# bcosm/CantorRL

Hardware: AMD Instinct MI355X
Metric: env-steps/sec (batched episodes) (higher is better)
Workload: dtype f64+f32; 1 GPU; configs[1]: 65,536 parallel envs/GPU, European call (BS rolling-ATM marks), GBM, v2 env, train_ppo_v2 reward; config_index=2, envs_per_gpu=65536, episode_length=252, mode=rollout, rollout_k=256, action_sets=1, parallelism=env-shard x1

## Files before the change

### cantorrl_amd/csrc/hedge_env.hip

```cpp
#include <hip/hip_runtime.h>
#include <hip/hip_ext.h>

#include <math.h>
#include <stdarg.h>
#include <stdio.h>
#include <stdlib.h>
#include <string.h>

#include <chrono>
#include <new>
#include <type_traits>

#include "vn_moments.h"
#include <string>
#include <vector>

#include "../../include/hedge_env.h"
#include "he_math.h"

using namespace he;

namespace {

#define GLOBAL __attribute__((address_space(1)))
// ... 1623 lines not shown
                                                          int slot0, vn::MomentsArgs vm) {
    Io io;
    io.act = sio.act;
    io.obs = sio.obs;
    io.rew = sio.rew;
    io.term = sio.term;
    io.trunc = sio.trunc;
    io.tobs = sio.tobs;
    io.info = he_info{};
    io.pol_on = false;
    io.sums = false;
    io.sig = nullptr;
    static_assert(kEpw == 64 && kEpb == kBlock, "one env per thread");
    const int64_t r = (int64_t)blockIdx.x * kEpb + threadIdx.x;
    const double ret_prev = (vm.upd_ret && r < n) ? vm.returns[r] : 0.0;
    const double col_shift = vn::load_col_shift(vm);
    VnHook hk{nullptr, 0.0f, 0.0, false};
    step_body<MODE, false, true, BOOK, FAST, false, GS>(*pc, n, tA, tB, tC, s, io, 1, slot0, blockIdx.x, &hk);
    __syncthreads();
    vn::moments_from_rows(vm, blockIdx.x, hk.tile, hk.rew, ret_prev, col_shift);
}

template <int MODE, bool BOOK, bool FAST, bool GS>
__global__ __launch_bounds__(kBlock) void step1_vne_kernel(const Params* __restrict__ pc, int64_t n, const float4* tA,
                                                           const float4* tB, const double* tC, State s, StepIo sio,
                                                           int slot0, vn::ApplyArgs va) {
    Io io;
    io.act = sio.act;
    io.obs = sio.obs;
    io.rew = sio.rew;
    io.term = sio.term;
    io.trunc = sio.trunc;
    io.tobs = sio.tobs;
    io.info = he_info{};
    io.pol_on = false;
    io.sums = false;
    io.sig = nullptr;
    static_assert(kEpw == 64 && kEpb == kBlock, "one env per thread");
    const int64_t r0 = (int64_t)blockIdx.x * kEpb;
    __shared__ vn::FrozenNorm fz;
    const vn::FrozenPre fp = vn::load_frozen(va, r0 + threadIdx.x, r0 + threadIdx.x < n);
    vn::prep_frozen(fz, va, fp);
    VnHook hk{nullptr, 0.0f, 0.0, false};
    step_body<MODE, false, true, BOOK, FAST, false, GS>(*pc, n, tA, tB, tC, s, io, 1, slot0, blockIdx.x, &hk);
    const int rows = (int)((n - r0) < kEpb ? n - r0 : kEpb);
    __syncthreads();
    vn::apply_frozen_rows(va, fz, r0, rows, hk.tile, fp, hk.rew, hk.rew64, hk.term, sio.tobs);
}

__global__ __launch_bounds__(vn::kVnThreads) void vn_moments_after_step_kernel(vn::MomentsArgs vm) {
    vn::moments_body(vm, blockIdx.x);
}

constexpr int kFusedWaves = kMktWaves;
template <int MODE, bool BOOK, bool FAST, bool GS>
__global__ __launch_bounds__(kBlock, kFusedWaves) void step_market_kernel(const Params* __restrict__ pc, int32_t buf,
                                                                           State s, Io io, int k_steps, int slot0,
                                                                           Market cur, Market bak,
                                                                           int32_t step_blocks) {
    static_assert(kBlock == kMktEnvs * kMktLanes, "one workgroup shape for both roles");
    if ((int32_t)blockIdx.x < step_blocks) {
        const Params& pk = pc[buf];
        step_body<MODE, false, false, BOOK, FAST, false, GS>(pk, pk.n, pk.tileA, pk.tileB, pk.tileC, s, io, k_steps,
                                                              slot0, blockIdx.x);
    } else {
        market_body<MODE, BOOK>(pc[buf ^ 1], cur, bak, 0, (int64_t)blockIdx.x - step_blocks);
    }
}

#ifndef HE_LDS_BALANCE
#define HE_LDS_BALANCE 1
#endif


constexpr int kPrioRewBook = 0, kPrioReplayRew = 0, kPrioObs = 2, kPrioProd = 1;
constexpr int kPrioGbmRew = 3, kPrioGbmObs = 2, kPrioGbmProd0 = 1, kPrioGbmProd1 = 0;
constexpr int kLdsLanesGbm = 2, kLdsLanesBook = 2, kLdsMinWavesBook = 4;
constexpr int kLdsEnvs = 64;
constexpr int kLdsM = 8;
constexpr int kLdsPrefetch = kLdsM % 6 == 0 ? 6 : (kLdsM % 4 == 0 ? 4 : kLdsM);
static_assert(kLdsM % kLdsPrefetch == 0, "the action ring index is the slot mod D");

template <int MODE, bool BOOK>
struct LdsGeom {
    static constexpr bool HESTON = MODE == HE_MODE_HESTON;
    static constexpr int lanes = (BOOK || HESTON) ? kLdsLanesBook : kLdsLanesGbm;
    static constexpr int prod = lanes;
    static constexpr int penvs = kLdsEnvs / lanes;
    static constexpr int threads = 64 * (2 + prod);
    static constexpr int H = kLdsM / lanes;
    static constexpr int minwaves = (BOOK || HESTON) ? kLdsMinWavesBook
                                                     : (HE_LDS_BALANCE ? 4 : (4 * (2 + prod) + 3) / 4 + 1);
    static_assert(H * lanes == kLdsM && penvs * lanes == kLdsEnvs, "producer lane layout");
};

constexpr int kLdsBookRows = 256;
constexpr int lds_thp_rows() { return 512; }
template <int MODE, bool BOOK, bool LEAN = false>
struct LdsMarketT {
    static constexpr int NB = 2;
    static constexpr bool THP = LEAN && !BOOK;
    double thp[THP ? lds_thp_rows() : 1];
    float2 sc[NB][kLdsM][kLdsEnvs];
    float pp[NB][kLdsM][kLdsEnvs];
    float stage[2][kLdsEnvs * kObs];
    double bk[BOOK ? 2 : 1][BOOK ? kLdsM : 1][kLdsEnvs];
    float vv[MODE == HE_MODE_HESTON ? 2 : 1][MODE == HE_MODE_HESTON ? kLdsM : 1][kLdsEnvs];
    double btab[BOOK ? kLdsBookRows : 1][4];
    BookOpt bopt[BOOK ? HE_BOOK_MAX : 1];
    uint32_t tame[NB][2];
};
static_assert(kLdsM > 8 || sizeof(LdsMarketT<HE_MODE_GBM, false>) <= 40 * 1024, "4 workgroups per CU");
static_assert(kLdsM > 8 || sizeof(LdsMarketT<HE_MODE_GBM, false, true>) <= 40 * 1024 - 64, "4 workgroups per CU");
static_assert(kLdsM > 8 || sizeof(LdsMarketT<HE_MODE_HESTON, true>) <= 40 * 1024, "4 workgroups per CU");

#ifdef HE_LDS_TIMING
__device__ uint64_t g_lds_tim[4][4096][5];
#define LDS_T0() uint64_t tim_t0 = __builtin_amdgcn_s_memtime(), tim_bar = 0, tim_r0 = __builtin_amdgcn_s_memrealtime()
#define LDS_BAR()                                                  \
    do {                                                           \
        const uint64_t tb_ = __builtin_amdgcn_s_memtime();         \
        __syncthreads();                                           \
        tim_bar += __builtin_amdgcn_s_memtime() - tb_;             \
    } while (0)
#define LDS_T1(role)                                                                     \
    do {                                                                                 \
        if ((threadIdx.x & 63) == 0 && blockIdx.x < 4096) {                              \
            g_lds_tim[role][blockIdx.x][0] = __builtin_amdgcn_s_memtime() - tim_t0;      \
            g_lds_tim[role][blockIdx.x][1] = tim_bar;                                    \
            const uint64_t r1_ = __builtin_amdgcn_s_memrealtime();                       \
            g_lds_tim[role][blockIdx.x][2] = r1_ - tim_r0;                               \
            g_lds_tim[role][blockIdx.x][3] = tim_r0;                                     \
            g_lds_tim[role][blockIdx.x][4] = r1_;                                        \
        }                                                                                \
    } while (0)
#else
#define LDS_T0() do {} while (0)
#define LDS_BAR() __syncthreads()
#define LDS_T1(role) do {} while (0)
#endif

__device__ __forceinline__ void flush_obs_full(const float* img, float* out, int64_t row0, int lane) {
    asm volatile("" ::: "memory");
    GLOBAL float* dst = (GLOBAL float*)out + row0 * kObs;
    GLOBAL v4f* d4 = (GLOBAL v4f*)dst;
    const v4f* s4 = reinterpret_cast<const v4f*>(img);
    d4[lane] = s4[lane];
    d4[lane + 64] = s4[lane + 64];
    d4[lane + 128] = s4[lane + 128];
    dst[768 + lane] = img[768 + lane];
    asm volatile("" ::: "memory");
}

template <int MODE, bool BOOK, bool LEAN, bool OBS, bool POL = false, bool PLAIN_OK = false, bool TAME_OK = false>
__device__ __forceinline__ void lds_stepper(const Params& p, State s, const Io& io, int k_steps, const Market& cur,
                                            LdsMarketT<MODE, BOOK, LEAN>& L, int64_t base) {
    constexpr int D = kLdsPrefetch;
    constexpr bool HESTON = MODE == HE_MODE_HESTON;
    const int lane = threadIdx.x & 63;
    const int64_t N = p.n;
    const int nfull = k_steps / kLdsM;
    const int tail = k_steps - nfull * kLdsM;
    const int64_t i0 = base + lane;
    const int64_t i = i0 < N ? i0 : N - 1;
    const int wrows = (int)((N - base) < kLdsEnvs ? (N - base) : kLdsEnvs);
    const Mkt rst{p.rstv[0], p.rstv[1], p.rstv[2], p.rstv[3], BOOK ? p.book_rst : 0.0};
    const GLOBAL v2f* gact = (const GLOBAL v2f*)io.act;
    GLOBAL float* const grew = (GLOBAL float*)io.rew;
    GLOBAL uint8_t* const gterm = (GLOBAL uint8_t*)io.term;
    if (!BOOK && !HESTON) {
        if (OBS) __builtin_amdgcn_s_setprio(kPrioGbmObs);
        else __builtin_amdgcn_s_setprio(kPrioGbmRew);
    } else {
        if (OBS) __builtin_amdgcn_s_setprio(kPrioObs);
        else __builtin_amdgcn_s_setprio(kPrioRewBook);
    }
    LDS_T0();
    Env e{};
    Mkt pre = rst;
    double pv_last = 0.0;
    {
        const uint32_t t0 = s.t[i];
        const uint32_t pk = s.pos[i];
        e.t = t0;
        e.call = unpack_lo(pk);
        e.put = unpack_hi(pk);
        e.path = -1;
        e.s0_small = rst.S < 1e-6f;
        e.s0 = e.s0_small ? 1.0f : rst.S;
        if (!OBS) {
            e.cash = s.cash[i];
            if (t0 != 0) {
                const double Sc = cur.S[i];
                const double Vc = HESTON ? cur.v[i] : p.var;
                const double Bc = BOOK ? book_value(p, Sc, Vc, (int32_t)t0, cur.M[i]) : 0.0;
                pre = Mkt{(float)Sc, HESTON ? (float)Vc : p.var_f, cur.C[i], cur.P[i], Bc};
            }
            pv_last = portfolio_value<BOOK>(p, e, pre);
        }
    }
    double sm0 = 0.0, sm1 = 0.0, sm2 = 0.0;
    uint32_t slen = 0;
    float last0 = 0.f, last1 = 0.f, last2 = 0.f, last3 = 0.f;
    if (!OBS) {
        sm0 = s.sum[i];
        sm1 = s.sum[N + i];
        sm2 = s.sum[2 * N + i];
        slen = s.sum_len[i];
        last0 = s.last[i];
        last1 = s.last[N + i];
        last2 = s.last[2 * N + i];
        last3 = s.last[3 * N + i];
    }
    auto account = [&](double reward, double pnl, double tc, bool term) {
        const double a0 = sm0 + reward, a1 = sm1 + pnl, a2 = sm2 + tc;
        const uint32_t n = slen + 1u;
        float f0 = (float)a0, f1 = (float)a1, f2 = (float)a2, f3 = (float)n;
        asm volatile("" : "+v"(f0), "+v"(f1), "+v"(f2), "+v"(f3));
        last0 = term ? f0 : last0;
        last1 = term ? f1 : last1;
        last2 = term ? f2 : last2;
        last3 = term ? f3 : last3;
        sm0 = term ? 0.0 : a0;
        sm1 = term ? 0.0 : a1;
        sm2 = term ? 0.0 : a2;
        slen = term ? 0u : n;
    };
    float2 ra[D];
    if constexpr (!POL) {
#pragma unroll
        for (int d = 0; d < D; ++d) ra[d] = ld2(gact, (int64_t)(d < k_steps ? d : k_steps - 1) * N + i);
    } else {
#pragma unroll
        for (int d = 0; d < D; ++d) ra[d] = make_float2(0.0f, 0.0f);
    }
    const int pol = POL ? io.pol.policy : HE_POLICY_NO_HEDGE;
    const bool pol_greeks = POL && pol != HE_POLICY_NO_HEDGE;
    float po3 = 0.0f, po4 = 0.0f, pcd = 0.0f, ppd = 0.0f;
    double acc[7] = {0.0, 0.0, 0.0, 0.0, 0.0, 0.0, 0.0};
    uint32_t acc_len = 0;
    const bool pmh = LEAN || p.maxh != 0, prm = LEAN || p.record_metrics;
    if constexpr (POL) {
        po3 = pmh ? div_int_byf((float)e.call, p.maxh_f, p.inv_maxh_f) : 0.0f;
        po4 = pmh ? div_int_byf((float)e.put, p.maxh_f, p.inv_maxh_f) : 0.0f;
        if (e.t == 0) {
            pcd = p.rstv[4 + 7];
            ppd = p.rstv[4 + 9];
        } else if (pol_greeks && prm) {
            const float S0f = (float)cur.S[i];
            float4 g0;
            if constexpr (!LEAN) g0 = greeks_fast<!HESTON>(p, S0f, HESTON ? (float)cur.v[i] : p.var_f);
            else if constexpr (HESTON) g0 = greeks_fast<false>(p, S0f, (float)cur.v[i]);
            else g0 = greeks_lean(S0f, p.g_num_drift, p.g_inv_sst_f, p.g_sst_f);
            pcd = g0.x;
            ppd = g0.z;
        }
        if (!OBS) {
#pragma unroll
            for (int c = 0; c < 7; ++c) acc[c] = s.acc[(int64_t)c * N + i];
            acc_len = s.acc_len[i];
        }
    }
    auto pol_account = [&](double reward, double pnl, double ps, double tc, double rpc, double tcp, bool term) {
        acc[0] = acc[0] + reward;
        acc[1] = acc[1] + pnl;
        acc[2] = acc[2] + fabs(ps);
        acc[3] = acc[3] + tc;
        acc[4] = acc[4] + rpc;
        acc[5] = acc[5] + tcp;
        acc[6] = acc[6] + ps;
        acc_len += 1u;
        if (__ballot(term) != 0ull) {
            if (term) {
                if (i0 < N) {
                    const unsigned long long r = atomicAdd(io.pol.count, 1ull);
                    if ((int64_t)r < io.pol.cap) {
                        he_episode_record rec;
                        rec.env_id = p.goff + i;
                        rec.length = (int32_t)acc_len;
                        rec.reserved = 0;
                        rec.reward_sum = acc[0];
                        rec.pnl_sum = acc[1];
                        rec.abs_pnl_sum = acc[2];
                        rec.cost_sum = acc[3];
                        rec.pnl_penalty_sum = acc[4];
                        rec.cost_penalty_sum = acc[5];
                        rec.per_share_pnl_sum = acc[6];
                        rec.reserved2 = 0.0;
                        io.pol.rec[r] = rec;
                    }
                }
                last0 = (float)acc[0];
                last1 = (float)acc[1];
                last2 = (float)acc[3];
                last3 = (float)acc_len;
#pragma unroll
                for (int c = 0; c < 7; ++c) acc[c] = 0.0;
                acc_len = 0;
            }
        }
    };

    constexpr int NB = LdsMarketT<MODE, BOOK, LEAN>::NB;
    constexpr bool kPlain = PLAIN_OK && LEAN && !POL;
    constexpr bool kTame = kPlain && TAME_OK && OBS && MODE == HE_MODE_GBM && !BOOK;
    const bool tame_h = kTame && p.lds_tame != 0;
    auto run_blk = [&](auto&& step, auto&& pre_ok) {
        LDS_BAR();
        for (int b = 0; b < nfull; ++b) {
            const int buf = b % NB;
            auto slots = [&](auto plain) {
#pragma unroll
                for (int sl = 0; sl < kLdsM; ++sl) {
                    const int k = b * kLdsM + sl;
                    const float2 ak = ra[sl % D];
                    if constexpr (!POL) {
                        const int kn = k + D;
                        ra[sl % D] = ld2(gact, (int64_t)(kn < k_steps ? kn : k_steps - 1) * N + i);
                    }
                    step(buf, sl, k, ak, std::true_type{}, plain);
                }
            };
            if constexpr (kPlain) {
                if (__ballot((int32_t)(e.t + (uint32_t)kLdsM) >= p.T) == 0ull) {
                    if constexpr (kTame) {
                        const uint32_t tw = __builtin_amdgcn_readfirstlane(L.tame[buf][0] & L.tame[buf][1]);
                        if (tame_h && tw != 0u && __ballot(!pre_ok()) == 0ull) slots(std::integral_constant<int, 2>{});
                        else slots(std::true_type{});
                    } else {
                        slots(std::true_type{});
                    }
                } else {
                    slots(std::false_type{});
                }
            } else {
                slots(std::false_type{});
            }
            LDS_BAR();
        }
        if (tail) {
            const int buf = nfull % NB;
            for (int sl = 0; sl < tail; ++sl) {
                const int k = nfull * kLdsM + sl;
                step(buf, sl, k, POL ? make_float2(0.0f, 0.0f) : ld2(gact, (int64_t)k * N + i), std::false_type{},
                     std::false_type{});
            }
            LDS_BAR();
        }
    };

    if constexpr (LEAN) {
        const float mt_f = p.mt_f, maxh_f = p.maxh_f, inv_maxh_f = p.inv_maxh_f;
        const int32_t mt = p.mt, maxh = p.maxh, T = p.T;
        if (OBS) {
            const float s0s_f = p.s0s_f, inv_s0s_f = p.inv_s0s_f;
            const float T_f = p.T_f, inv_T_f = p.inv_T_f, var_f = p.var_f;
            const float gnd = p.g_num_drift, gis = p.g_inv_sst_f, gsf = p.g_sst_f;
            float ro[kObs];
#pragma unroll
            for (int c = 0; c < kObs; ++c) ro[c] = p.rstv[4 + c];
            float preS = pre.S;
            if (e.t != 0) preS = (float)cur.S[i];
            const float dv12 = np_clipf(var_f - var_f, -1.0f, 1.0f);
            auto pre_ok = [&] { return preS >= 64.0f && preS <= 8388608.0f; };
            float preV = rst.v;
            if (HESTON && e.t != 0) preV = (float)cur.v[i];
            const double s0s_d = p.s0s_d, inv_s0s_d = p.inv_s0s_d;
            using lds_float = __attribute__((address_space(3))) float;
            lds_float* row0 = (lds_float*)&L.stage[0][lane * kObs];
            lds_float* row1 = (lds_float*)&L.stage[1][lane * kObs];
            asm volatile("" : "+v"(row0), "+v"(row1));
            auto obs_step = [&](int buf, int sl, int k, float2 ak, auto full, auto plain) {
                constexpr bool PLAIN = decltype(plain)::value;
                constexpr bool TAME = (int)decltype(plain)::value == 2;
                const float2 r0 = L.sc[buf][sl][lane];
                const float rP = L.pp[buf][sl][lane];
                const float vk = HESTON ? L.vv[HESTON ? buf : 0][HESTON ? sl : 0][lane] : var_f;
                float4 g;
                if constexpr (HESTON) g = greeks_fast<false>(p, r0.x, vk);
                else g = greeks_lean_t<TAME>(r0.x, gnd, gis, gsf);
                if constexpr (POL) {
                    ak = policy_action(p, pol, e.call, e.put, po3, po4, pcd, ppd);
                    if (io.pol.act_out) {
                        v2f av = {ak.x, ak.y};
                        ((GLOBAL v2f*)io.pol.act_out)[(int64_t)k * N + i] = av;
                    }
                }
                const int32_t nc = e.call + trade_round(ak.x * mt_f, mt);
                const int32_t nq = e.put + trade_round(ak.y * mt_f, mt);
                const int32_t cc = clamp_pos(nc, maxh);
                const int32_t qq = clamp_pos(nq, maxh);
                const uint32_t t1 = e.t + 1;
                const bool term = !PLAIN && (int32_t)t1 >= T;
                float o[kObs];
                if constexpr (TAME) {
                    o[0] = div_f32_byf_nz(r0.x, s0s_f, inv_s0s_f);
                    o[1] = div_f32_by_nz(r0.y, s0s_d, inv_s0s_d);
                    o[2] = div_f32_by_nz(rP, s0s_d, inv_s0s_d);
                } else {
                    if constexpr (HESTON) {
                        o[0] = div_f32_by(r0.x, s0s_d, inv_s0s_d);
                    } else {
                        o[0] = div_f32_byf(r0.x, s0s_f, inv_s0s_f);
                    }
                    o[1] = div_f32_by(r0.y, s0s_d, inv_s0s_d);
                    o[2] = div_f32_by(rP, s0s_d, inv_s0s_d);
                }
                o[3] = div_int_byf((float)cc, maxh_f, inv_maxh_f);
                o[4] = div_int_byf((float)qq, maxh_f, inv_maxh_f);
                o[5] = vk;
                o[6] = div_int_byf((float)(T - (int32_t)t1), T_f, inv_T_f);
                o[7] = g.x;
                o[8] = g.y;
                o[9] = g.z;
                o[10] = g.y;
                o[11] = lag_return_lean<TAME>(r0.x, preS);
                if constexpr (HESTON) o[12] = (preS == 0.0f) ? 0.0f : np_clipf(vk - preV, -1.0f, 1.0f);
                else if constexpr (TAME) o[12] = 0.0f;
                else o[12] = (preS == 0.0f) ? 0.0f : dv12;
                float* const tile = L.stage[k & 1];
                lds_float* const row = (k & 1) ? row1 : row0;
#pragma unroll
                for (int c = 0; c < kObs; ++c) row[c] = o[c];
                if constexpr (!PLAIN) {
                    if (__ballot(term) != 0ull) {
                        if (term) {
#pragma unroll
                            for (int c = 0; c < kObs; ++c) row[c] = ro[c];
                        }
                    }
                }
                if (!POL || io.obs) {
                    float* out = io.obs + (int64_t)k * N * kObs;
                    if constexpr (decltype(full)::value) flush_obs_full(tile, out, base, lane);
                    else flush_obs_wave(tile, out, base, wrows, lane);
                }
                if constexpr (POL) {
                    po3 = term ? ro[3] : o[3];
                    po4 = term ? ro[4] : o[4];
                    pcd = term ? ro[7] : o[7];
                    ppd = term ? ro[9] : o[9];
                }
                e.t = term ? 0u : t1;
                e.call = term ? 0 : cc;
                e.put = term ? 0 : qq;
                preS = term ? rst.S : r0.x;
                if (HESTON) preV = term ? rst.v : vk;
            };
            if (wrows == kLdsEnvs)
                run_blk([&](int buf, int sl, int k, float2 ak, auto, auto plain) {
                    obs_step(buf, sl, k, ak, std::true_type{}, plain);
                }, pre_ok);
            else
                run_blk([&](int buf, int sl, int k, float2 ak, auto, auto plain) {
                    obs_step(buf, sl, k, ak, std::false_type{}, plain);
                }, pre_ok);
        } else {
            const double tcpc = p.tcpc, slip_frac = p.slip_frac, lam = p.lam, w = p.w, theta = p.theta;
            const double shares_d = p.shares_d, inv_shares = p.inv_shares, den = p.den, inv_den = p.inv_den;
            const double inv_252 = p.inv_252, init_cash = p.initial_cash;
// ... 370 lines not shown
                        if (BOOK) Mr = np_max(Mr, S);
                        if (!PLAIN) tp = (tp + 1 == T) ? 0u : tp + 1;
                    }
#pragma unroll
                    for (int h = 0; h < kLdsH; ++h) Sx[h] = (j == sl0 + h) ? S : Sx[h];
                    if (BOOK) {
#pragma unroll
                        for (int h = 0; h < kLdsH; ++h) Mx[h] = (j == sl0 + h) ? Mr : Mx[h];
                    }
                }
            }
            Sbs = S;
            if (BOOK) Mbs = Mr;
            uint32_t tp = tpf;
            const int wb = bp % LdsMarketT<MODE, BOOK, LEAN>::NB;
            double lkC[kLdsH], lkP[kLdsH];
            if constexpr (LOCK) {
                double Sm[kLdsH], Km[kLdsH];
                uint32_t tq = tpf;
#pragma unroll
                for (int h = 0; h < kLdsH; ++h) {
                    if constexpr (PLAIN) {
                        Sm[h] = Sx[h];
                    } else {
                        const bool last = tq + 1 == T;
                        const double Sprev = (h == 0) ? Sin : Sx[h - 1];
                        Sm[h] = last ? ((tq == 0) ? p.s0 : Sprev) : Sx[h];
                        tq = (tq + 1 == T) ? 0u : tq + 1;
                    }
                    Km[h] = rint(Sm[h]);
                }
                bs_call_put_n<kLdsH>(Sm, Km, p.bs, lkC, lkP);
            }
            if constexpr (kTame) {
                uint32_t verdict = 0u;
                if constexpr (LOCK && PLAIN) {
                    uint32_t smin = (uint32_t)__double2hiint(Sx[0]), smax = smin;
                    uint32_t mmin = (uint32_t)__double2hiint(lkC[0]), mmax = mmin;
#pragma unroll
                    for (int h = 0; h < kLdsH; ++h) {
                        const uint32_t sh = (uint32_t)__double2hiint(Sx[h]);
                        const uint32_t ch = (uint32_t)__double2hiint(lkC[h]), ph = (uint32_t)__double2hiint(lkP[h]);
                        smin = sh < smin ? sh : smin;
                        smax = sh > smax ? sh : smax;
                        mmin = ch < mmin ? ch : mmin;
                        mmax = ch > mmax ? ch : mmax;
                        mmin = ph < mmin ? ph : mmin;
                        mmax = ph > mmax ? ph : mmax;
                    }
                    const bool ok = smin >= 0x40500000u && smax < 0x41600000u && mmin >= 0x38100000u && mmax < 0x47e00000u;
                    verdict = __ballot(!ok) == 0ull ? 0xffffffffu : 0u;
                }
                W.tame[wb][pw] = verdict;
            }
            if constexpr (LOCK) {
#pragma unroll
                for (int h = 0; h < kLdsH; ++h) {
                    const int sl = sl0 + h;
                    W.sc[wb][sl][le] = make_float2((float)Sx[h], (float)lkC[h]);
                    W.pp[wb][sl][le] = (float)lkP[h];
                }
            } else {
                double rS[kLdsH], rV[kLdsH];
#pragma unroll
                for (int h = 0; h < kLdsH; ++h) {
                    rS[h] = Sx[h];
                    rV[h] = HESTON ? Vx[h] : p.var;
                }
                double Sprev = Sin, Vprev = Vin;
#pragma unroll 1
                for (int h = 0; h < kLdsH; ++h) {
                    if (FULL || sl0 + h < len) {
                        const bool last = tp + 1 == T;
                        const double Sm = last ? ((tp == 0) ? p.s0 : Sprev) : rS[0];
                        const double Vh = rV[0];
                        const double Vm = HESTON ? (last ? ((tp == 0) ? p.var : Vprev) : Vh) : p.var;
                        float C, P;
                        marks<MODE, !LEAN>(p, Sm, Vm, last ? tp : tp + 1u, &C, &P);
                        const int sl = sl0 + h;
                        W.sc[wb][sl][le] = make_float2((float)rS[0], C);
                        W.pp[wb][sl][le] = P;
                        if (HESTON) W.vv[HESTON ? wb : 0][HESTON ? sl : 0][le] = (float)Vh;
                        tp = (tp + 1 == T) ? 0u : tp + 1;
                    }
                    Sprev = rS[0];
                    Vprev = rV[0];
#pragma unroll
                    for (int q = 0; q + 1 < kLdsH; ++q) {
                        rS[q] = rS[q + 1];
                        rV[q] = rV[q + 1];
                    }
                }
            }
            if constexpr (BOOK) {
                double bS[kLdsH], bV[kLdsH], bM[kLdsH];
#pragma unroll
                for (int h = 0; h < kLdsH; ++h) {
                    bS[h] = Sx[h];
                    bV[h] = HESTON ? Vx[h] : p.var;
                    bM[h] = Mx[h];
                }
                uint32_t tb = tpf;
#pragma unroll 1
                for (int h = 0; h < kLdsH; ++h) {
                    if (HESTON) prod_prio_toggle((h + pw) & 1);
                    else prod_prio_toggle(pw == 1 ? (h != 3) : (h == 3));
                    if (FULL || sl0 + h < len)
                        W.bk[wb][sl0 + h][le] = book_value<!HESTON>(p, bS[0], bV[0], (int32_t)(tb + 1), bM[0],
                                                                    &W.btab[0][0], &W.bopt[0]);
                    tb = (tb + 1 == T) ? 0u : tb + 1;
#pragma unroll
                    for (int q = 0; q + 1 < kLdsH; ++q) {
                        bS[q] = bS[q + 1];
                        bV[q] = bV[q + 1];
                        bM[q] = bM[q + 1];
                    }
                }
            }
            };
            if (len == kLdsM) {
                if constexpr (PLAIN_OK && LEAN && !HESTON && !BOOK) {
                    if (__ballot(tpb == 0u || tpb + (uint32_t)kLdsM >= T) == 0ull)
                        block(std::true_type{}, std::true_type{});
                    else
                        block(std::true_type{}, std::false_type{});
                } else {
                    block(std::true_type{}, std::false_type{});
                }
            } else {
                block(std::false_type{}, std::false_type{});
            }
            tpb = episode_wrap(tpb, (uint32_t)kLdsM, T);
        }
        LDS_BAR();
    }
    if (nb > 0 && sub == 0) {
        const int sll = (k_steps - 1) - (nb - 1) * kLdsM;
        const int wbl = (nb - 1) % LdsMarketT<MODE, BOOK, LEAN>::NB;
        int64_t j = pi;
        asm volatile("" : "+v"(j));
        const uint32_t ep0 = cur.ep[j], t0 = cur.t[j];
        const uint32_t q = (t0 >= T ? T : t0) + (uint32_t)(k_steps - 1);
        cur.ep[j] = ep0 + q / T;
        cur.t[j] = q % T + 1u;
        cur.S[j] = Sbs;
        if (HESTON) cur.v[j] = Vbs;
        cur.C[j] = W.sc[wbl][sll][le].y;
        cur.P[j] = W.pp[wbl][sll][le];
        if (BOOK) cur.M[j] = Mbs;
    }
    LDS_T1(2 + (pw < 2 ? pw : 1));
}

#if HE_LDS_BALANCE || defined(HE_LDS_HWID)
__device__ uint32_t g_cu_ticket[4096];
#endif
#ifdef HE_LDS_HWID
__device__ uint32_t g_lds_hwid[16384][4][4];
#endif
__device__ __forceinline__ uint32_t hw_cu_key(uint32_t hw, uint32_t xcc) {
    return ((xcc & 15u) << 8) | (((hw >> 13) & 7u) << 5) | (((hw >> 12) & 1u) << 4) | ((hw >> 8) & 15u);
}
template <int NWAVES>
__device__ __forceinline__ int lds_role(int wave) {
#if HE_LDS_BALANCE || defined(HE_LDS_HWID)
    if constexpr (NWAVES == 4) {
        __shared__ uint32_t sh_place[5];
        const uint32_t hw = __builtin_amdgcn_s_getreg((31 << 11) | 4);
        const uint32_t xcc = __builtin_amdgcn_s_getreg((15 << 11) | 20);
        const uint32_t simd = (hw >> 4) & 3u;
        if ((threadIdx.x & 63) == 0) sh_place[wave] = simd;
        if (threadIdx.x == 0) sh_place[4] = atomicAdd(&g_cu_ticket[hw_cu_key(hw, xcc & 15u)], 1u);
        __syncthreads();
        const uint32_t m = (1u << sh_place[0]) | (1u << sh_place[1]) | (1u << sh_place[2]) | (1u << sh_place[3]);
        int role = wave;
#if HE_LDS_BALANCE
        if (m == 15u) role = (int)((simd + sh_place[4]) & 3u);
#endif
#ifdef HE_LDS_HWID
        if ((threadIdx.x & 63) == 0 && blockIdx.x < 16384) {
            g_lds_hwid[blockIdx.x][wave][0] = hw;
            g_lds_hwid[blockIdx.x][wave][1] = xcc;
            g_lds_hwid[blockIdx.x][wave][2] = sh_place[4];
            g_lds_hwid[blockIdx.x][wave][3] = (uint32_t)role | (m << 8);
        }
#endif
        return __builtin_amdgcn_readfirstlane(role);
    }
#endif
    return wave;
}

constexpr int kLdsNumSgpr = 96;
constexpr bool kPlainPersistS = false, kPlainPersistP = true;
template <int MODE, bool BOOK, bool LEAN, bool PERSIST = false, bool POL = false>
__global__ __launch_bounds__((LdsGeom<MODE, BOOK>::threads), (LdsGeom<MODE, BOOK>::minwaves))
    __attribute__((amdgpu_num_sgpr(kLdsNumSgpr))) void lds_rollout_kernel(const Params* __restrict__ pc, State s, Io io,
                                                                 int k_steps, Market cur) {
    __shared__ __attribute__((aligned(16))) LdsMarketT<MODE, BOOK, LEAN> lm;
    const Params& p = *pc;
    const int wave = lds_role<LdsGeom<MODE, BOOK>::threads / 64>(__builtin_amdgcn_readfirstlane(threadIdx.x >> 6));
    if constexpr (BOOK) {
        const int nv = 4 * p.book_rows;
        for (int k = threadIdx.x; k < nv; k += LdsGeom<MODE, BOOK>::threads) (&lm.btab[0][0])[k] = p.book_tab[k];
        if ((int)threadIdx.x < p.book_n) lm.bopt[threadIdx.x] = p.book[threadIdx.x];
        __syncthreads();
    }
    if constexpr (!PERSIST) {
        const int64_t base = (int64_t)blockIdx.x * kLdsEnvs;
        if (wave == 0) lds_stepper<MODE, BOOK, LEAN, false, POL, true>(p, s, io, k_steps, cur, lm, base);
        else if (wave == 1) lds_stepper<MODE, BOOK, LEAN, true, POL, true, !POL>(p, s, io, k_steps, cur, lm, base);
        else lds_producer<MODE, BOOK, LEAN, true, !POL>(p, k_steps, cur, lm, base, wave - 2);
        return;
    }
    const int64_t tiles = (p.n + kLdsEnvs - 1) / kLdsEnvs;
    for (int64_t tile = blockIdx.x; tile < tiles; tile += gridDim.x) {
        asm volatile("" ::: "memory");
        const int64_t base = tile * kLdsEnvs;
        if (wave == 0) lds_stepper<MODE, BOOK, LEAN, false, POL, kPlainPersistS>(p, s, io, k_steps, cur, lm, base);
        else if (wave == 1) lds_stepper<MODE, BOOK, LEAN, true, POL, kPlainPersistS>(p, s, io, k_steps, cur, lm, base);
        else lds_producer<MODE, BOOK, LEAN, kPlainPersistP>(p, k_steps, cur, lm, base, wave - 2);
        if (tile + gridDim.x < tiles) __syncthreads();
    }
}

struct LdsReplay {
    float4 mk[2][kLdsM][kLdsEnvs];
    float2 gd[2][kLdsM][kLdsEnvs];
    float gg[2][kLdsM][kLdsEnvs];
    float4 rk[2][kLdsEnvs];
    float4 rg[2][kLdsEnvs];
    float stage[2][kLdsEnvs * kObs];
};
static_assert(kLdsM > 8 || sizeof(LdsReplay) <= 40 * 1024 - 64, "4 workgroups per CU");

__device__ __forceinline__ void lds_replay_loader(const Params& p, State s, int k_steps, LdsReplay& L,
                                                  int64_t base, int part) {
    constexpr int H = kLdsM / 2;
    static_assert(kLdsM == 8, "two lanes per env, 4 slots each: one 128-B line of rows per block");
    const int lane = threadIdx.x & 63;
    const int hh = lane >> 5;
    const int le = part * 32 + (lane & 31);
    const int64_t N = p.n;
    const int64_t i0 = base + le;
    const int64_t i = i0 < N ? i0 : N - 1;
    const uint32_t T = (uint32_t)p.T;
    const int64_t W = p.rstride;
    const GLOBAL v4f* rec = (const GLOBAL v4f*)p.rec;
    const GLOBAL v4f* recg = (const GLOBAL v4f*)p.recg;
    const int sl0 = hh * H;
    __builtin_amdgcn_s_setprio(kPrioProd);
    LDS_T0();
    int32_t path = s.path[i];
    uint32_t t = s.t[i];
    Pcg64 g;
    g.sh = s.pcg[i];
    g.sl = s.pcg[N + i];
    g.ih = s.pcg[2 * N + i];
    g.il = s.pcg[3 * N + i];
    g.has32 = s.pcgb[i];
    g.buf32 = s.pcgb[N + i];
    float s0enc = s.s0[i];
    const int nb = (k_steps + kLdsM - 1) / kLdsM;
    float4 A[H], B[H];
    float4 Y[H];
    bool hand = false;
    float4 R0 = make_float4(0.f, 0.f, 0.f, 0.f), G0 = R0;
    int rsl = kLdsM;
    auto issue = [&](int bp) {
        const int kb = bp * kLdsM;
        const int len = (k_steps - kb) < kLdsM ? (k_steps - kb) : kLdsM;
        const bool take = hand;
        if (__ballot(take) != 0ull) {
#pragma unroll
            for (int h = 0; h < H; ++h) {
                Y[h].x = __shfl(Y[h].x, lane | 32);
                Y[h].y = __shfl(Y[h].y, lane | 32);
                Y[h].z = __shfl(Y[h].z, lane | 32);
                Y[h].w = __shfl(Y[h].w, lane | 32);
            }
        }
        const uint32_t te = T - 1u - t;
        rsl = te < (uint32_t)len ? (int)te : kLdsM;
        int32_t np = path;
        if (rsl < kLdsM) np = (int32_t)pcg64_integers(g, (uint64_t)p.n_paths);
        const int64_t ro = (int64_t)path * W + p.roff + (int64_t)t + 1, rn = (int64_t)np * W + p.roff;
        hand = rsl == kLdsM && (ro & 7) == 4 && t + 12u <= T;
        if (hh == 0 && take) {
#pragma unroll
            for (int h = 0; h < H; ++h) A[h] = Y[h];
        } else {
#pragma unroll
            for (int h = 0; h < H; ++h) {
                const int sl = sl0 + h;
                const int64_t r = (sl <= rsl) ? ro + sl : rn + (sl - rsl);
                A[h] = ld4(rec, r);
            }
        }
        if (hh == 1 && hand) {
#pragma unroll
            for (int h = 0; h < H; ++h) Y[h] = ld4(rec, ro + kLdsM + h);
        }
        if (hh == 0 && rsl < kLdsM) {
            R0 = ld4(rec, rn);
            G0 = ld4(recg, rn);
        }
        if (rsl < kLdsM) {
            path = np;
            t = (uint32_t)(len - 1 - rsl);
        } else {
            t += (uint32_t)len;
        }
    };
    if (nb > 0) issue(0);
    for (int bp = 0; bp <= nb; ++bp) {
        if (bp < nb) {
            const int kb = bp * kLdsM;
            const int len = (k_steps - kb) < kLdsM ? (k_steps - kb) : kLdsM;
            const int wb = bp & 1;
#pragma unroll
            for (int h = 0; h < H; ++h) {
                const int sl = sl0 + h;
                if (sl < len) {
                    B[h] = p.record_metrics ? replay_greeks(p, A[h].x, A[h].y) : make_float4(0.f, 0.f, 0.f, 0.f);
                    L.mk[wb][sl][le] = A[h];
                    L.gd[wb][sl][le] = make_float2(B[h].x, B[h].z);
                    L.gg[wb][sl][le] = B[h].y;
                }
            }
            if (hh == 0) {
                L.rk[wb][le] = R0;
                L.rg[wb][le] = G0;
                if (rsl < kLdsM) s0enc = (R0.x < 1e-6f) ? -1.0f : R0.x;
            }
            if (bp + 1 < nb) issue(bp + 1);
        }
        LDS_BAR();
    }
    LDS_T1(2 + part);
    if (hh == 0 && i0 < N) {
        int64_t j = i;
        asm volatile("" : "+v"(j));
        s.path[j] = path;
        s.s0[j] = s0enc;
        s.pcg[j] = g.sh;
        s.pcg[N + j] = g.sl;
        s.pcgb[j] = g.has32;
        s.pcgb[N + j] = g.buf32;
    }
}

__device__ __forceinline__ uint32_t fresh_lane() {
    uint32_t ln;
    asm volatile("v_mbcnt_lo_u32_b32 %0, -1, 0\n\tv_mbcnt_hi_u32_b32 %0, -1, %0" : "=v"(ln));
    return ln;
}

template <bool OBS, bool FAST, bool POL = false>
__device__ __forceinline__ void lds_replay_stepper(const Params& p, State s, const Io& io, int k_steps,
                                                   LdsReplay& L, int64_t base) {
    constexpr int D = kLdsPrefetch;
    static_assert(kLdsM % D == 0, "the action ring index is the slot mod D");
    const int lane = threadIdx.x & 63;
    const int64_t N = p.n;
    const int nfull = k_steps / kLdsM;
// ... 1938 lines not shown
```

Baseline: 65.73 billion env-steps/s.

## Split GBM LDS producer into pipelined factor-generation and marks-pricing waves

For the plain GBM non-book lean rollout, the two producer waves are replaced by a two-stage pipeline. One wave generates Philox normals and exp growth factors into a double-buffered LDS stage. The other wave consumes those factors to advance the price and compute Black-Scholes marks into the market LDS buffers. The stepper waves take an extra barrier to stay aligned with the deeper pipeline. This aims to overlap RNG/exp work with pricing, at the cost of extra LDS, an extra barrier stage, and a possible occupancy loss.

```diff
diff --git a/cantorrl_amd/csrc/hedge_env.hip b/cantorrl_amd/csrc/hedge_env.hip
--- a/cantorrl_amd/csrc/hedge_env.hip
+++ b/cantorrl_amd/csrc/hedge_env.hip
@@ -1799,7 +1799,8 @@
     asm volatile("" ::: "memory");
 }
 
-template <int MODE, bool BOOK, bool LEAN, bool OBS, bool POL = false, bool PLAIN_OK = false, bool TAME_OK = false>
+template <int MODE, bool BOOK, bool LEAN, bool OBS, bool POL = false, bool PLAIN_OK = false, bool TAME_OK = false,
+          bool STAGE = false>
 __device__ __forceinline__ void lds_stepper(const Params& p, State s, const Io& io, int k_steps, const Market& cur,
                                             LdsMarketT<MODE, BOOK, LEAN>& L, int64_t base) {
     constexpr int D = kLdsPrefetch;
@@ -1953,6 +1954,7 @@
     constexpr bool kTame = kPlain && TAME_OK && OBS && MODE == HE_MODE_GBM && !BOOK;
     const bool tame_h = kTame && p.lds_tame != 0;
     auto run_blk = [&](auto&& step, auto&& pre_ok) {
+        if constexpr (STAGE) LDS_BAR();
         LDS_BAR();
         for (int b = 0; b < nfull; ++b) {
             const int buf = b % NB;
@@ -2629,6 +2631,210 @@
     LDS_T1(2 + (pw < 2 ? pw : 1));
 }
 
+struct LdsStageGf {
+    double gf[2][kLdsM][kLdsEnvs];
+};
+static_assert(kLdsM > 8 || sizeof(LdsMarketT<HE_MODE_GBM, false, true>) + sizeof(LdsStageGf) <= 40 * 1024 - 64,
+              "4 workgroups per CU");
+#ifdef HE_LDS_STAGE_PRIO_SWAP
+constexpr int kPrioStageFactors = kPrioGbmProd0, kPrioStageMarks = kPrioGbmProd1;
+#else
+constexpr int kPrioStageFactors = kPrioGbmProd1, kPrioStageMarks = kPrioGbmProd0;
+#endif
+
+__device__ __forceinline__ void lds_stage_factors(const Params& p, int k_steps, const Market& cur, LdsStageGf& G,
+                                                  int64_t base) {
+    static_assert(kLdsM == 8, "4 Philox blocks (5 from an odd step index) per block of 8 slots");
+    const int lane = threadIdx.x & 63;
+    const int64_t N = p.n;
+    const int nb = (k_steps + kLdsM - 1) / kLdsM;
+    const int64_t pi = (base + lane) < N ? base + lane : N - 1;
+    __builtin_amdgcn_s_setprio(kPrioStageFactors);
+    uint64_t a0;
+    {
+        const uint32_t T = (uint32_t)p.T;
+        const uint32_t ep0 = cur.ep[pi], t0 = cur.t[pi];
+        a0 = (uint64_t)ep0 * T + (t0 >= T ? T : t0);
+    }
+    LDS_T0();
+    for (int bf = 0; bf <= nb + 1; ++bf) {
+        if (bf < nb) {
+            const int64_t gid = p.goff + pi;
+            const uint64_t nf = a0 + (uint64_t)(bf * kLdsM);
+            const uint64_t m0 = nf >> 1;
+            const bool odd = (nf & 1) != 0;
+            double zs[kLdsM];
+            if (__ballot(odd) == 0ull) {
+                philox_normals_n<kLdsM / 2>(p, gid, m0, zs);
+            } else {
+                double zz[kLdsM + 2];
+                philox_normals_n<kLdsM / 2 + 1>(p, gid, m0, zz);
+#pragma unroll
+                for (int j = 0; j < kLdsM; ++j) {
+                    double a = zz[j], b = zz[j + 1];
+                    asm volatile("" : "+v"(a), "+v"(b));
+                    zs[j] = odd ? b : a;
+                }
+            }
+            double arg[kLdsM], ex[kLdsM];
+#pragma unroll
+            for (int j = 0; j < kLdsM; ++j) {
+                const double dW = p.sqrt_dt * zs[j];
+                arg[j] = p.drift + p.sqrt_var * dW;
+            }
+            exp_k_n<4>(arg, ex);
+            exp_k_n<4>(arg + 4, ex + 4);
+            const int wb = bf & 1;
+#pragma unroll
+            for (int j = 0; j < kLdsM; ++j) G.gf[wb][j][lane] = ex[j];
+        }
+        LDS_BAR();
+    }
+    LDS_T1(2);
+}
+
+__device__ __forceinline__ void lds_stage_marks(const Params& p, int k_steps, const Market& cur,
+                                                LdsMarketT<HE_MODE_GBM, false, true>& W, const LdsStageGf& G,
+                                                int64_t base) {
+    constexpr int NB = LdsMarketT<HE_MODE_GBM, false, true>::NB;
+    constexpr int kHalf = kLdsM / 2;
+    const int lane = threadIdx.x & 63;
+    const int64_t N = p.n;
+    const int nb = (k_steps + kLdsM - 1) / kLdsM;
+    const uint32_t T = (uint32_t)p.T;
+    const int64_t pi = (base + lane) < N ? base + lane : N - 1;
+    __builtin_amdgcn_s_setprio(kPrioStageMarks);
+    uint32_t tpb;
+    {
+        const uint32_t t0 = cur.t[pi];
+        tpb = t0 >= T ? 0u : t0;
+    }
+    double Sbs = cur.S[pi];
+    LDS_T0();
+    LDS_BAR();
+    for (int bp = 0; bp <= nb; ++bp) {
+        if (bp < nb) {
+            const int kb = bp * kLdsM;
+            const int len = (k_steps - kb) < kLdsM ? (k_steps - kb) : kLdsM;
+            const int wb = bp % NB;
+            auto block = [&](auto full, auto plain) {
+                constexpr bool FULL = decltype(full)::value;
+                constexpr bool PLAIN = decltype(plain)::value;
+                double eall[kLdsM];
+#pragma unroll
+                for (int j = 0; j < kLdsM; ++j) eall[j] = G.gf[bp & 1][j][lane];
+                const double Sin = Sbs;
+                double Sa[kLdsM];
+                double S = Sbs;
+                uint32_t tp = tpb;
+#pragma unroll
+                for (int j = 0; j < kLdsM; ++j) {
+                    if (FULL || j < len) {
+                        if (!PLAIN && tp == 0) S = p.s0;
+                        const double Sn = S * eall[j];
+                        S = (Sn < 1e-8) ? 1e-8 : Sn;
+                        if (!PLAIN) tp = (tp + 1 == T) ? 0u : tp + 1;
+                    }
+                    Sa[j] = S;
+                }
+                Sbs = S;
+                if constexpr (FULL) {
+                    uint32_t smin = 0xffffffffu, smax = 0u, mmin = 0xffffffffu, mmax = 0u;
+                    uint32_t tq = tpb;
+#pragma unroll
+                    for (int h0 = 0; h0 < kLdsM; h0 += kHalf) {
+                        double Sm[kHalf], Km[kHalf], lkC[kHalf], lkP[kHalf];
+#pragma unroll
+                        for (int h = 0; h < kHalf; ++h) {
+                            const int j = h0 + h;
+                            if constexpr (PLAIN) {
+                                Sm[h] = Sa[j];
+                            } else {
+                                const bool last = tq + 1 == T;
+                                const double Sprev = (j == 0) ? Sin : Sa[j == 0 ? 0 : j - 1];
+                                Sm[h] = last ? ((tq == 0) ? p.s0 : Sprev) : Sa[j];
+                                tq = (tq + 1 == T) ? 0u : tq + 1;
+                            }
+                            Km[h] = rint(Sm[h]);
+                        }
+                        bs_call_put_n<kHalf>(Sm, Km, p.bs, lkC, lkP);
+#pragma unroll
+                        for (int h = 0; h < kHalf; ++h) {
+                            const int j = h0 + h;
+                            if constexpr (PLAIN) {
+                                const uint32_t sh = (uint32_t)__double2hiint(Sa[j]);
+                                const uint32_t ch = (uint32_t)__double2hiint(lkC[h]), ph = (uint32_t)__double2hiint(lkP[h]);
+                                smin = sh < smin ? sh : smin;
+                                smax = sh > smax ? sh : smax;
+                                mmin = ch < mmin ? ch : mmin;
+                                mmax = ch > mmax ? ch : mmax;
+                                mmin = ph < mmin ? ph : mmin;
+                                mmax = ph > mmax ? ph : mmax;
+                            }
+                            W.sc[wb][j][lane] = make_float2((float)Sa[j], (float)lkC[h]);
+                            W.pp[wb][j][lane] = (float)lkP[h];
+                        }
+                    }
+                    uint32_t verdict = 0u;
+                    if constexpr (PLAIN) {
+                        const bool ok = smin >= 0x40500000u && smax < 0x41600000u && mmin >= 0x38100000u && mmax < 0x47e00000u;
+                        verdict = __ballot(!ok) == 0ull ? 0xffffffffu : 0u;
+                    }
+                    W.tame[wb][0] = verdict;
+                    W.tame[wb][1] = verdict;
+                } else {
+                    double rS[kLdsM];
+#pragma unroll
+                    for (int j = 0; j < kLdsM; ++j) rS[j] = Sa[j];
+                    double Sprev = Sin;
+                    uint32_t tm = tpb;
+#pragma unroll 1
+                    for (int j = 0; j < kLdsM; ++j) {
+                        if (j < len) {
+                            const bool last = tm + 1 == T;
+                            const double Sm = last ? ((tm == 0) ? p.s0 : Sprev) : rS[0];
+                            float C, P;
+                            marks<HE_MODE_GBM, false>(p, Sm, p.var, last ? tm : tm + 1u, &C, &P);
+                            W.sc[wb][j][lane] = make_float2((float)rS[0], C);
+                            W.pp[wb][j][lane] = P;
+                            tm = (tm + 1 == T) ? 0u : tm + 1;
+                        }
+                        Sprev = rS[0];
+#pragma unroll
+                        for (int q = 0; q + 1 < kLdsM; ++q) rS[q] = rS[q + 1];
+                    }
+                    W.tame[wb][0] = 0u;
+                    W.tame[wb][1] = 0u;
+                }
+            };
+            if (len == kLdsM) {
+                if (__ballot(tpb == 0u || tpb + (uint32_t)kLdsM >= T) == 0ull)
+                    block(std::true_type{}, std::true_type{});
+                else
+                    block(std::true_type{}, std::false_type{});
+            } else {
+                block(std::false_type{}, std::false_type{});
+            }
+            tpb = episode_wrap(tpb, (uint32_t)kLdsM, T);
+        }
+        LDS_BAR();
+    }
+    if (nb > 0) {
+        const int sll = (k_steps - 1) - (nb - 1) * kLdsM;
+        const int wbl = (nb - 1) % NB;
+        int64_t j = pi;
+        asm volatile("" : "+v"(j));
+        const uint32_t ep0 = cur.ep[j], t0 = cur.t[j];
+        const uint32_t q = (t0 >= T ? T : t0) + (uint32_t)(k_steps - 1);
+        cur.ep[j] = ep0 + q / T;
+        cur.t[j] = q % T + 1u;
+        cur.S[j] = Sbs;
+        cur.C[j] = W.sc[wbl][sll][lane].y;
+        cur.P[j] = W.pp[wbl][sll][lane];
+    }
+    LDS_T1(3);
+}
+
 #if HE_LDS_BALANCE || defined(HE_LDS_HWID)
 __device__ uint32_t g_cu_ticket[4096];
 #endif
@@ -2685,9 +2891,18 @@
     }
     if constexpr (!PERSIST) {
         const int64_t base = (int64_t)blockIdx.x * kLdsEnvs;
-        if (wave == 0) lds_stepper<MODE, BOOK, LEAN, false, POL, true>(p, s, io, k_steps, cur, lm, base);
-        else if (wave == 1) lds_stepper<MODE, BOOK, LEAN, true, POL, true, !POL>(p, s, io, k_steps, cur, lm, base);
-        else lds_producer<MODE, BOOK, LEAN, true, !POL>(p, k_steps, cur, lm, base, wave - 2);
+        constexpr bool kStage = MODE == HE_MODE_GBM && !BOOK && LEAN && !POL;
+        if constexpr (kStage) {
+            __shared__ __attribute__((aligned(16))) LdsStageGf gf;
+            if (wave == 0) lds_stepper<MODE, BOOK, LEAN, false, POL, true, false, true>(p, s, io, k_steps, cur, lm, base);
+            else if (wave == 1) lds_stepper<MODE, BOOK, LEAN, true, POL, true, true, true>(p, s, io, k_steps, cur, lm, base);
+            else if (wave == 2) lds_stage_factors(p, k_steps, cur, gf, base);
+            else lds_stage_marks(p, k_steps, cur, lm, gf, base);
+        } else {
+            if (wave == 0) lds_stepper<MODE, BOOK, LEAN, false, POL, true>(p, s, io, k_steps, cur, lm, base);
+            else if (wave == 1) lds_stepper<MODE, BOOK, LEAN, true, POL, true, !POL>(p, s, io, k_steps, cur, lm, base);
+            else lds_producer<MODE, BOOK, LEAN, true, !POL>(p, k_steps, cur, lm, base, wave - 2);
+        }
         return;
     }
     const int64_t tiles = (p.n + kLdsEnvs - 1) / kLdsEnvs;
```

Result: no change. 65.79 billion env-steps/s (median of 2 runs) (+0.1%).
